# nz0001na/MorphGANformer

Hardware: AMD Instinct MI355X
Metric: latent-projection iters/sec @1024^2, k=17 latents (higher is better)
Workload: dtype f32; 1 GPU; configs[1]: single 1024x1024 face per GPU, Wing+LPIPS(squeeze)+MSE literal-mode projection step, noise_mode=random, seeded synthetic weights/targets/landmarks; k=17, z_dim=32, targets_per_gpu=1, parallelism=pair-sharded x1, graph_replay=True, loss_generator_overlap=True, steps_per_forward=32

## Files before the change

### include/mgf.h

```cpp
#ifndef MGF_H_
#define MGF_H_

#include <stdint.h>

#ifdef __cplusplus
extern "C" {
#endif

typedef void* mgf_stream_t;

enum { MGF_OK = 0, MGF_EINVAL = -1, MGF_EUNSUPPORTED = -2, MGF_ELAUNCH = -3, MGF_ETOOBIG = -4 };
enum { MGF_F32 = 0, MGF_F64 = 1, MGF_F16 = 2 };
enum { MGF_FILTER_SEPARABLE = 2 };
enum { MGF_FILTER_LARGE = 4 };
enum { MGF_ACT_LINEAR = 1, MGF_ACT_RELU = 2, MGF_ACT_LRELU = 3, MGF_ACT_TANH = 4, MGF_ACT_SIGMOID = 5,
       MGF_ACT_ELU = 6, MGF_ACT_SELU = 7, MGF_ACT_SOFTPLUS = 8, MGF_ACT_SWISH = 9,
       MGF_ACT_RELU_POST = 10 };

const char* mgf_last_error(void);
int mgf_version(void);
int mgf_device_ok(void);

int mgf_bias_act(void* y, const void* x, const void* b, const void* xref, const void* yref, const void* dy,
                 int dtype, int64_t numel, int64_t step_b, int64_t size_b,
// ... 121 lines not shown
} mgf_style_job;
int mgf_demod_f32(float* d, const float* s, const float* wsq, int32_t n, int32_t cin, int32_t cout, mgf_stream_t stream);
int mgf_demod_bwd_f32(float* ds, const float* dd, const float* d, const float* s, const float* wsq, int32_t n, int32_t cin, int32_t cout,
                      mgf_stream_t stream);
int mgf_style_demod(const mgf_style_job* job, const float* ws, int64_t ws_stride_n, int32_t n, int32_t wdim, mgf_stream_t stream);
int mgf_style_demod_multi(const mgf_style_job* jobs_dev, int32_t njobs, const float* ws, int64_t ws_stride_n,
                          int32_t n, int32_t wdim, int32_t max_cin, mgf_stream_t stream);

int mgf_duplex_attention(float* y, const float* x, const float* wqc, const float* spos, const float* vwb,
                         int32_t n, int32_t c, int32_t f, int32_t t,
                         const mgf_epilogue* ep, int32_t ep_w, float* probs, int32_t* argmax, mgf_stream_t stream);

int mgf_att_map_upsample_f32(float* out, const float* probs, int32_t n, int32_t side, int32_t t, int32_t out_res, int32_t layer,
                             int32_t n_layers, mgf_stream_t stream);

typedef struct mgf_attn_job {
    const float* wmv;
    const float* bmv;
    float* vwb;
    int32_t c;
    int32_t w_offset;
} mgf_attn_job;
int mgf_attn_values(const mgf_attn_job* job, const float* ws, int64_t ws_stride_n, int64_t ws_stride_t, int32_t n, int32_t t,
                    int32_t wdim, mgf_stream_t stream);
int mgf_attn_values_multi(const mgf_attn_job* jobs_dev, int32_t njobs, const float* ws, int64_t ws_stride_n, int64_t ws_stride_t,
                          int32_t n, int32_t t, int32_t wdim, mgf_stream_t stream);

int mgf_randn_f32(float* out, int64_t n, uint64_t seed, void* state, mgf_stream_t stream);
int mgf_rgb_weights_f32(float* out, const float* w, const float* s, int32_t n, int32_t c, int32_t cout, mgf_stream_t stream);
int mgf_torgb_compose_weights_f32(float* w_eff, const float* w_last, const float* s_last, const float* d_last, const float* w_rgb,
                                  const float* s_rgb, int32_t n, int32_t cin, int32_t cout, int32_t rgb_channels, mgf_stream_t stream);
int mgf_conv3x3_few_outputs_f32(float* y, const float* x, const float* w, const float* bias, int32_t n, int32_t cin, int32_t h, int32_t wd,
                                int32_t cout, mgf_stream_t stream);

int64_t mgf_mapping_param_floats(int32_t k, int32_t dim, int32_t n_res_layers);
int mgf_mapping_forward(float* w, const float* z, const float* params, int32_t n, int32_t k, int32_t dim,
                        int32_t n_res_layers, int32_t normalize_global, mgf_stream_t stream);

int64_t mgf_reduce_scratch_floats(void);
int mgf_mse_f32(float* out, const float* a, const float* b, int32_t n, int64_t numel, int64_t b_batch_stride, float scale,
                int32_t accumulate, float* scratch, mgf_stream_t stream);
int64_t mgf_dssim_scratch_bytes(int32_t n, int32_t c, int32_t h, int32_t w);
int mgf_dssim_u8_f32(float* out, const float* img, const float* target, int32_t n, int32_t c, int32_t h, int32_t w, int64_t t_batch_stride,
                     float data_range, float scale, int32_t accumulate, void* scratch, mgf_stream_t stream);
int mgf_dssim_f32(float* out, const float* img, const float* target, int32_t n, int32_t c, int32_t h, int32_t w, int64_t t_batch_stride,
                  float data_range, float scale, int32_t accumulate, void* scratch, mgf_stream_t stream);
int mgf_dssim_grad_f32(float* dimg, float* out, const float* img, const float* target, int32_t n, int32_t c, int32_t h, int32_t w,
                       int64_t t_batch_stride, float data_range, float scale, int32_t accumulate_dimg, int32_t accumulate_out, void* scratch,
                       mgf_stream_t stream);
int64_t mgf_msssim_scratch_bytes(int32_t n, int32_t c, int32_t h, int32_t w, int32_t levels);
int mgf_msssim_f32(float* out, const float* img, const float* target, int32_t n, int32_t c, int32_t h, int32_t w, int64_t t_batch_stride,
                   const double* weights, int32_t levels, float data_range, float scale, int32_t accumulate, void* scratch, mgf_stream_t stream);
int mgf_msssim_grad_f32(float* dimg, float* out, const float* img, const float* target, int32_t n, int32_t c, int32_t h, int32_t w,
                        int64_t t_batch_stride, const double* weights, int32_t levels, float data_range, float scale, int32_t accumulate_dimg,
                        int32_t accumulate_out, void* scratch, mgf_stream_t stream);
int64_t mgf_lbp_scratch_bytes(int32_t n);
int mgf_lbp_gray224_u8(uint8_t* gray, const float* img, const int32_t* tables, int32_t n, int32_t h, int32_t w, int32_t true_rgb_order,
                       mgf_stream_t stream);
int mgf_lbp_codes_u8(uint8_t* codes, const uint8_t* gray, const double* offsets, int32_t n, mgf_stream_t stream);
int mgf_lbp_distance_f64(double* out, const uint8_t* gray, const uint8_t* target_codes, const double* offsets, int32_t n, void* scratch,
                         mgf_stream_t stream);
int mgf_wing_loss_f64(double* out, const double* pred, const double* target, int32_t n, int64_t numel, double omega, double epsilon,
                      const int32_t* pred_step, int32_t max_row, mgf_stream_t stream);
int mgf_adaptive_wing_loss_f64(double* out, const double* pred, const double* target, int32_t n, int64_t numel, double omega, double theta,
                               double epsilon, double alpha, const int32_t* pred_step, int32_t max_row, mgf_stream_t stream);
int mgf_embed_pair_loss_f32(float* loss, float* demb, double* trace, const float* emb, const float* ta, const float* tb, const float* alpha,
// ... 199 lines not shown
```

### morphganformer_amd/_lib.py

```python
from __future__ import annotations

import ctypes as C
import os

import torch

HERE = os.path.dirname(os.path.abspath(__file__))
LIB_PATH = os.environ.get("MGF_LIB_PATH") or os.path.join(HERE, "libmgf_hip.so")

MGF_F32, MGF_F64, MGF_F16 = 0, 1, 2
ACT_IDS = {"linear": 1, "relu": 2, "lrelu": 3, "tanh": 4, "sigmoid": 5, "elu": 6, "selu": 7, "softplus": 8, "swish": 9,
           "relu_post": 10}
MAX_TAPS = 9

i32, i64, f32, f64, vp = C.c_int32, C.c_int64, C.c_float, C.c_double, C.c_void_p


class Epilogue(C.Structure):
    _fields_ = [("bias", vp), ("noise", vp), ("noise_strength", vp), ("noise_n", i32), ("act", i32), ("alpha", f32),
                ("gain", f32), ("residual", vp)]


class ConvDesc(C.Structure):
    _fields_ = [("n", i32), ("cin", i32), ("in_h", i32), ("in_w", i32), ("cout", i32), ("cout_pad", i32),
# ... 44 lines not shown
    "mgf_tconv3x3s2_blur_f32": (C.c_int, [vp, vp, vp, vp, vp, vp, C.c_float, i32, i32, i32, i32, i32, i32, i64, i64, i64, i64, C.POINTER(Epilogue), vp]),
    "mgf_tconv3x3s2_winograd_f32": (C.c_int, [vp, vp, vp, vp, vp, i32, i32, i32, i32, i32, i32, i64, i64, i64, vp]),
    "mgf_tconv_winograd_weights_f32": (C.c_int, [vp, vp, i32, i32, C.c_double, vp]),
    "mgf_winograd_weights_f32": (C.c_int, [vp, vp, i32, i32, f32, vp]),
    "mgf_conv3x3_winograd_f32": (C.c_int, [vp, vp, vp, vp, vp, i32, i32, i32, i32, i32, i32, C.POINTER(Epilogue), vp]),
    "mgf_winograd2_weights_f32": (C.c_int, [vp, vp, i32, i32, f32, vp]),
    "mgf_conv3x3_winograd2_f32": (C.c_int, [vp, vp, vp, vp, vp, i32, i32, i32, i32, i32, i32, C.POINTER(Epilogue), vp]),
    "mgf_conv3x3_winograd2_rgb_f32": (C.c_int, [vp, vp, vp, vp, vp, vp, vp, i32, i32, i32, i32, i32, i32, i32, vp]),
    "mgf_conv3x3_winograd3_f32": (C.c_int, [vp, vp, vp, vp, vp, i32, i32, i32, i32, i32, i32, C.POINTER(Epilogue), vp]),
    "mgf_conv1x1_f32": (C.c_int, [vp, vp, vp, vp, i32, i32, i32, i32, i32, i64, i32, C.POINTER(Epilogue), vp]),
    "mgf_conv3x3s2_few_inputs_f32": (C.c_int, [vp, vp, vp, vp, i32, i32, i32, i32, i32, i32, vp]),
    "mgf_tconv3x3s2_few_outputs_f32": (C.c_int, [vp, vp, vp, i32, i32, i32, i32, i32, i32, i32, i64, i64, vp]),
    "mgf_conv1x1_force_shape": (C.c_int, [i32]),
    "mgf_conv3x3_winograd3_slice_f32": (C.c_int, [vp, vp, vp, vp, vp, i32, i32, i32, i32, i32, i32, i64, i32, C.POINTER(Epilogue), vp]),
    "mgf_conv3x3_winograd3_up2res_f32": (C.c_int, [vp, vp, vp, vp, vp, vp, i32, i32, i32, i32, i32, i32, C.POINTER(Epilogue), vp]),
    "mgf_winograd3_force_shape": (C.c_int, [i32]),
    "mgf_conv3x3_winograd3_rgb_f32": (C.c_int, [vp, vp, vp, vp, vp, vp, vp, i32, i32, i32, i32, i32, i32, i32, vp]),
    "mgf_conv3x3_winograd2_slice_f32": (C.c_int, [vp, vp, vp, vp, vp, i32, i32, i32, i32, i32, i32, i64, i32, C.POINTER(Epilogue), vp]),
    "mgf_pack_conv_weights": (C.c_int, [vp, vp, vp, i32, i32, i32, i32, i32, f32, i32, vp]),
    "mgf_conv_profile_begin": (C.c_int, []),
    "mgf_conv_profile_end": (C.c_int, [C.POINTER(ConvProfRec), i32]),
    "mgf_demod_f32": (C.c_int, [vp, vp, vp, i32, i32, i32, vp]),
    "mgf_demod_bwd_f32": (C.c_int, [vp, vp, vp, vp, vp, i32, i32, i32, vp]),
    "mgf_style_demod": (C.c_int, [C.POINTER(StyleJob), vp, i64, i32, i32, vp]),
    "mgf_style_demod_multi": (C.c_int, [vp, i32, vp, i64, i32, i32, i32, vp]),
    "mgf_duplex_attention": (C.c_int, [vp, vp, vp, vp, vp, i32, i32, i32, i32, C.POINTER(Epilogue), i32, vp, vp, vp]),
    "mgf_att_map_upsample_f32": (C.c_int, [vp, vp, i32, i32, i32, i32, i32, i32, vp]),
    "mgf_attn_values": (C.c_int, [C.POINTER(AttnJob), vp, i64, i64, i32, i32, i32, vp]),
    "mgf_attn_values_multi": (C.c_int, [vp, i32, vp, i64, i64, i32, i32, i32, vp]),
    "mgf_randn_f32": (C.c_int, [vp, i64, C.c_uint64, vp, vp]),
    "mgf_rgb_weights_f32": (C.c_int, [vp, vp, vp, i32, i32, i32, vp]),
    "mgf_torgb_compose_weights_f32": (C.c_int, [vp, vp, vp, vp, vp, vp, i32, i32, i32, i32, vp]),
    "mgf_conv3x3_few_outputs_f32": (C.c_int, [vp, vp, vp, vp, i32, i32, i32, i32, i32, vp]),
    "mgf_mapping_param_floats": (i64, [i32, i32, i32]),
    "mgf_mapping_forward": (C.c_int, [vp, vp, vp, i32, i32, i32, i32, i32, vp]),
    "mgf_reduce_scratch_floats": (i64, []),
    "mgf_mse_f32": (C.c_int, [vp, vp, vp, i32, i64, i64, f32, i32, vp, vp]),
    "mgf_dssim_scratch_bytes": (i64, [i32, i32, i32, i32]),
    "mgf_dssim_u8_f32": (C.c_int, [vp, vp, vp, i32, i32, i32, i32, i64, f32, f32, i32, vp, vp]),
    "mgf_dssim_f32": (C.c_int, [vp, vp, vp, i32, i32, i32, i32, i64, f32, f32, i32, vp, vp]),
    "mgf_dssim_grad_f32": (C.c_int, [vp, vp, vp, vp, i32, i32, i32, i32, i64, f32, f32, i32, i32, vp, vp]),
    "mgf_msssim_scratch_bytes": (i64, [i32, i32, i32, i32, i32]),
    "mgf_msssim_f32": (C.c_int, [vp, vp, vp, i32, i32, i32, i32, i64, vp, i32, f32, f32, i32, vp, vp]),
    "mgf_msssim_grad_f32": (C.c_int, [vp, vp, vp, vp, i32, i32, i32, i32, i64, vp, i32, f32, f32, i32, i32, vp, vp]),
    "mgf_lbp_scratch_bytes": (i64, [i32]),
    "mgf_lbp_gray224_u8": (C.c_int, [vp, vp, vp, i32, i32, i32, i32, vp]),
    "mgf_lbp_codes_u8": (C.c_int, [vp, vp, vp, i32, vp]),
    "mgf_lbp_distance_f64": (C.c_int, [vp, vp, vp, vp, i32, vp, vp]),
    "mgf_wing_loss_f64": (C.c_int, [vp, vp, vp, i32, i64, f64, f64, vp, i32, vp]),
    "mgf_adaptive_wing_loss_f64": (C.c_int, [vp, vp, vp, i32, i64, f64, f64, f64, f64, vp, i32, vp]),
    "mgf_embed_pair_loss_f32": (C.c_int, [vp, vp, vp, vp, vp, vp, vp, i32, i32, i64, f32, f32, i32, i32, vp, i32, vp]),
    "mgf_lpips_unit_f32": (C.c_int, [vp, vp, i32, i32, i64, vp]),
    "mgf_lpips_layer_f32": (C.c_int, [vp, vp, vp, vp, i32, i32, i64, i64, i32, vp, vp]),
    "mgf_lpips_stem_f32": (C.c_int, [vp, vp, vp, vp, vp, vp, vp, vp, i32, i32, i32, i32, vp, vp]),
    "mgf_lpips_layer_map_f32": (C.c_int, [vp, vp, vp, vp, i32, i32, i64, i64, vp]),
    "mgf_lpips_upsample_sum_f32": (C.c_int, [vp, C.POINTER(vp), C.POINTER(i32), i32, i32, i32, i32, vp]),
    "mgf_channel_affine_prelu_f32":(C.c_int, [vp, vp, vp, vp, vp, i32, i32, i64, vp]),
    "mgf_linear_f32": (C.c_int, [vp, vp, vp, vp, i32, i32, i32, vp]),
    "mgf_resize_bilinear_f32": (C.c_int, [vp, vp, i32, i32, i32, i32, i32, vp]),
    "mgf_spatial_mean_f32": (C.c_int, [vp, vp, i32, i64, vp]),
    "mgf_l2_normalize_f32": (C.c_int, [vp, vp, i32, i32, f32, vp]),
    "mgf_l2_normalize_bwd_f32": (C.c_int, [vp, vp, vp, i32, i32, f32, vp]),
    "mgf_spatial_mean_bwd_f32": (C.c_int, [vp, vp, i32, i64, vp]),
    "mgf_relu_bwd_slice_f32": (C.c_int, [vp, vp, i32, i32, vp, i32, i32, i32, i32, i64, vp]),
    "mgf_maxpool_s2_floor_f32": (C.c_int, [vp, vp, i32, i32, i32, i32, vp]),
    "mgf_maxpool3x3s2_ceil_f32": (C.c_int, [vp, vp, i32, i32, i32, i32, i32, vp]),
# ... 129 lines not shown
```

### morphganformer_amd/build.py

```python
from __future__ import annotations

import glob
import hashlib
import os
import subprocess
import sys

HERE = os.path.dirname(os.path.abspath(__file__))
ROOT = os.path.dirname(HERE)
CSRC = os.path.join(HERE, "csrc")
OBJ = os.path.join(CSRC, "_obj")
LIB = os.path.join(HERE, "libmgf_hip.so")
SOURCES = ["capi.cpp", "bias_act.hip", "upfirdn2d.hip", "conv_taps.hip", "latent_prep.hip", "attention.hip", "losses.hip", "lpips_stem.hip",
           "embed.hip", "backward.hip", "wino.hip", "wino3.hip", "pointwise.hip", "narrow_conv.hip", "warp.hip", "lbp.hip", "mdf.hip",
           "wino_tconv.hip", "depthwise.hip", "noise_opt.hip", "morph_pair.hip", "tconv_blur.hip", "msssim.hip"]
HEADERS = [os.path.join(CSRC, "mgf_common.h"), os.path.join(ROOT, "include", "mgf.h")]
HIPCC = os.environ.get("HIPCC", "/opt/rocm/bin/hipcc")
FLAGS = ["--offload-arch=gfx950", "-O3", "-fPIC", "-std=c++17", "-ffp-contract=on", "-Wno-unused-result", "-x", "hip"]
LINK_FLAGS = ["--offload-arch=gfx950", "-shared", "-fPIC"]

_compiler_id = None


def compiler_id() -> str:
    global _compiler_id
    if _compiler_id is None:
        _compiler_id = subprocess.run([HIPCC, "--version"], stdout=subprocess.PIPE, stderr=subprocess.STDOUT, check=True).stdout.decode()
    return _compiler_id


def object_key(src_path: str, flags) -> str:
    h = hashlib.sha256()
    h.update(compiler_id().encode())
    h.update("\0".join(flags).encode())
    for p in [src_path] + HEADERS:
        with open(p, "rb") as f:
            h.update(b"\0" + os.path.basename(p).encode() + b"\0" + f.read())
    return h.hexdigest()[:16]


def _compile_all(obj_dir, flags_for, verbose, force, prune=True):
    os.makedirs(obj_dir, exist_ok=True)
    objs, todo = [], []
    for src in SOURCES:
        sp = os.path.join(CSRC, src)
        flags = flags_for(src)
        op = os.path.join(obj_dir, f"{src}.{object_key(sp, flags)}.o")
        objs.append(op)
# ... 95 lines not shown
```

### morphganformer_amd/conv.py

```python
from __future__ import annotations

import ctypes as C
import os
from dataclasses import dataclass

import torch

from . import _lib


def round_up(v: int, m: int) -> int:
    return (v + m - 1) // m * m


def profile_begin():
    _lib.check(_lib.lib().mgf_conv_profile_begin(), "conv_profile_begin")


def profile_end(max_recs=4096):
    recs = (_lib.ConvProfRec * max_recs)()
    n = _lib.lib().mgf_conv_profile_end(recs, max_recs)
    if n < 0:
        _lib.check(n, "conv_profile_end")
    return [(recs[i].kernel.decode(), recs[i].flops, recs[i].seconds, recs[i].ksplit, recs[i].bytes) for i in range(min(n, max_recs))]


@dataclass
class PackedConv:
    wp: torch.Tensor
    wsq: torch.Tensor | None
    cout: int
    cin: int
    kh: int
    kw: int
    cout_pad: int
# ... 328 lines not shown

def tconv_pitch(w: int, align: int = 4) -> int:
    return round_up(2 * w + 1, align)


def conv3x3s2_few_inputs(x, w, bias=None, relu=False, out=None):
    _lib.require_gpu(x, w, bias, out)
    cout, cin = w.shape[:2]
    assert tuple(w.shape[2:]) == (3, 3) and cin <= 4 and w.is_contiguous() and w.dtype == torch.float32
    assert x.dtype == torch.float32 and x.is_contiguous() and x.shape[1] == cin
    n, _, h, wd = x.shape
    oh, ow = (h - 3) // 2 + 1, (wd - 3) // 2 + 1
    if out is None:
        out = torch.empty([n, cout, oh, ow], dtype=torch.float32, device=x.device)
    assert out.is_contiguous() and tuple(out.shape) == (n, cout, oh, ow)
    rc = _lib.lib().mgf_conv3x3s2_few_inputs_f32(out.data_ptr(), x.data_ptr(), w.data_ptr(), _lib.ptr(bias), n, cin, h, wd, cout, int(relu),
                                                 _lib.stream_ptr())
    _lib.check(rc, "conv3x3s2_few_inputs")
    return out


def conv3x3_few_outputs(x, w, bias=None, out=None):
    _lib.require_gpu(x, w, bias, out)
    n, cin, h, wd = x.shape
    cout = w.shape[1]
    assert x.dtype == torch.float32 and x.is_contiguous() and w.dtype == torch.float32 and w.is_contiguous()
    assert tuple(w.shape) == (n, cout, cin, 3, 3) and cout <= 4
    if out is None:
        out = torch.empty([n, cout, h, wd], dtype=torch.float32, device=x.device)
    assert out.is_contiguous() and tuple(out.shape) == (n, cout, h, wd)
    _lib.check(_lib.lib().mgf_conv3x3_few_outputs_f32(out.data_ptr(), x.data_ptr(), w.data_ptr(), _lib.ptr(bias), n, cin, h, wd, cout,
                                                      _lib.stream_ptr()), "conv3x3_few_outputs")
    return out


TCONV_WINO = os.environ.get("MGF_TCONV_WINO", "1") != "0"
TCONV_WINO_MIN_WGS = 4096


def tconv_winograd_weights(w: torch.Tensor, gain: float = 1.0) -> torch.Tensor:
    _lib.require_gpu(w)
    w = w.contiguous().float()
    cout, cin, kh, kw = w.shape
    assert (kh, kw) == (3, 3) and cin % 4 == 0
    u = torch.empty([25, cin // 4, cout, 4], dtype=torch.float32, device=w.device)
    _lib.check(_lib.lib().mgf_tconv_winograd_weights_f32(u.data_ptr(), w.data_ptr(), cout, cin, float(gain), _lib.stream_ptr()),
               "tconv_winograd_weights")
    return u


def tconv_winograd_ok(n, cin, h, w, cout, out, bf=None) -> bool:
    return bool(TCONV_WINO and SPLIT_TCONV_BORDER and bf is None and h % 2 == 0 and w % 2 == 0 and min(h, w) >= TCONV_SPLIT_MIN and cin % 4 == 0 and cout % 32 == 0
                and out.shape[3] % 4 == 0 and out.data_ptr() % 16 == 0
                and n * -(-h // 4) * -(-w // 32) * (cout // 32) >= TCONV_WINO_MIN_WGS)


def tconv3x3s2_forward(x, pc: PackedConv, in_scale=None, out_scale=None, out=None, bf=None, wt=None):
    _lib.require_gpu(x, pc.wp, in_scale, out_scale, out, wt)
    assert pc.kh == 3 and pc.kw == 3 and x.dtype == torch.float32 and x.is_contiguous()
    n, cin, h, w = x.shape
    oh, ow = 2 * h + 1, 2 * w + 1
    if out is None:
        out = torch.empty([n, pc.cout, oh, tconv_pitch(w)], dtype=torch.float32, device=x.device)
    pitch = out.shape[3]
    assert out.is_contiguous() and tuple(out.shape) == (n, pc.cout, oh, pitch) and pitch >= ow and pitch % 4 == 0
    if NARROW_CONV and pc.cout <= 4 and in_scale is None and out_scale is None:
# ... 106 lines not shown
```

### morphganformer_amd/engine.py

```python
from __future__ import annotations

import ctypes as C
import math
import os
from dataclasses import dataclass, field

import numpy as np
import torch

from . import _lib
from . import conv as cv
from .synth_weights import GeneratorConfig

SQRT2 = math.sqrt(2.0)
SQRT_HALF = math.sqrt(0.5)
USE_WINOGRAD = os.environ.get("MGF_WINOGRAD", "1") != "0"
WINOGRAD_MAX_RES = int(os.environ.get("MGF_WINOGRAD_MAX_RES", "1024"))
TCONV_WINO_MAX_RES = int(os.environ.get("MGF_TCONV_WINO_MAX_RES", "256"))
BF_DIRECT_MAX_RES = int(os.environ.get("MGF_BF_DIRECT_MAX_RES", "128"))


def pack_mapping_params(sd, cfg: GeneratorConfig) -> np.ndarray:
    D, T = cfg.w_dim, cfg.k - 1
    lr = cfg.mapping_lrmul
# ... 102 lines not shown
                lp.demod = False
            else:
                wg = 1.0 / math.sqrt(cin * 9)
                lp.pc = cv.pack_weights(t32(w), gain=wg, flip=False, want_wsq=True)
                if kind == "conv3" and USE_WINOGRAD and cv.winograd_ok(cin, cout, res, res) and res <= WINOGRAD_MAX_RES:
                    lp.wino_u = cv.winograd_pack(t32(w), wg, res)
                if (kind == "tconv" and arith != "bf16x3" and cv.TCONV_WINO and res <= TCONV_WINO_MAX_RES and cin % 4 == 0
                        and cout % 32 == 0):
                    lp.wino_t = cv.tconv_winograd_weights(t32(w), wg)
                if arith == "bf16x3" and cin % 16 == 0 and res // up >= 32:
                    lp.pcb = cv.pack_weights_bf16x3(lp.pc)
            lp.aff_w = t32(f64(p + ".affine.weight"))
            lp.aff_b = t32(f64(p + ".affine.bias"))
            if (p + ".biasAct.bias") in sd:
                lp.bias = t32(f64(p + ".biasAct.bias"))
            if (p + ".noise_strength") in sd:
                lp.noise_strength = t32(f64(p + ".noise_strength").reshape(1))
                lp.noise_const = t32(f64(p + ".noise_const"))
            lp.act_gain = SQRT2 * (SQRT_HALF if (name == "conv1" and res > 4) else 1.0)
            if att and (p + ".transformer.to_queries.weight") in sd:
                lp.attn = self._fold_attention(sd, p, cout, res, T, D, t32, f64)
                lp.attn.v_off = v_off
                v_off += cout * T
            if name == "conv_last" and lp.bias is None and lp.noise_strength is None and lp.attn is None and cfg.img_channels <= 4:
                lp.w_gained = t32(w / math.sqrt(cin * 9))
            lp.s_off, lp.d_off = s_off, d_off
            s_off += cin
            d_off += cout
            self.layers.append(lp)
        self.s_total, self.d_total, self.v_total = s_off, d_off, v_off
        for res in cfg.block_resolutions[1:]:
            w = f64(f"synthesis.b{res}.skip.weight")
            self.skips[res] = cv.pack_weights(t32(w), gain=SQRT_HALF / math.sqrt(w.shape[1]), flip=False)
        torch.cuda.synchronize(dev)

    @staticmethod
    def _fold_attention(sd, p, C_, res, T, D, t32, f64):
        tp = p + ".transformer"
        Fn = res * res
        wq = f64(tp + ".to_queries.weight") / math.sqrt(C_)
        bq = f64(tp + ".to_queries.bias")
        wfp = f64(tp + ".from_pos_map.weight") / math.sqrt(D)
        bfp = f64(tp + ".from_pos_map.bias")
        wv = f64(tp + ".to_values.weight") / math.sqrt(D)
        bv = f64(tp + ".to_values.bias")
        wm = f64(tp + ".modulation.weight") / math.sqrt(C_)
        bm = f64(tp + ".modulation.bias")
        aw = f64(tp + ".att_weight").reshape(2 * C_)
        cent = f64(tp + ".centroids").reshape(T, 2 * C_)
        a1 = cent[:, :C_] * aw[None, :C_]
        a2 = cent[:, C_:] * aw[None, C_:]
        inv = 1.0 / math.sqrt(C_)
        wqc = (wq.T @ a1.T) * inv
        pos_term = f64(p + ".grid_pos").reshape(Fn, D) @ wfp.T + bfp[None]
        spos = (pos_term @ a2.T + (bq @ a1.T)[None]) * inv
        wmv = wm @ wv
        bmv = wm @ bv + bm + 1.0
        return AttnPlan(c=C_, f=Fn, wqc=t32(wqc), spos=t32(spos), wmv=t32(wmv), bmv=t32(bmv))


class Generator:

    def __init__(self, sd, cfg: GeneratorConfig, device="cuda", max_batch: int = 1, arith: str = "f32"):
        if arith not in ("f32", "bf16x3"):
            raise ValueError(f"arith must be 'f32' or 'bf16x3' (got {arith!r})")
        self.cfg = cfg
        self.arith = arith
        self.tpitch_align = 32 if arith == "bf16x3" else 4
        self.plan = SynthesisPlan(sd, cfg, device, arith=arith)
        self.device = self.plan.device
        self.input_shape = [None, cfg.k, cfg.z_dim]
        self.cond_shape = [None, 0]
        self.z_dim, self.w_dim, self.k, self.c_dim = cfg.z_dim, cfg.w_dim, cfg.k, 0
        self.img_resolution, self.img_channels = cfg.img_resolution, cfg.img_channels
        self.num_ws = cfg.num_ws
        self.w_avg = torch.as_tensor(np.asarray(sd["mapping.w_avg"], dtype=np.float32), device=self.device)
        self._ws_cache = {}
        self.taps = None
        self.fuse_torgb = True
        self.skip_fused = {}
        self.fuse_skip_up = os.environ.get("MGF_FUSE_SKIP_UP", "1") != "0"
        self.last_noise = ("none", None)
        self.side = torch.cuda.Stream(device=self.device)
        self.overlap_skip = os.environ.get("MGF_OVERLAP_SKIP", "0") != "0"
        self.torgb_compose = os.environ.get("MGF_TORGB_COMPOSE", "1") != "0"
        self._workspaces, self._pins = {}, {}
        self.noise_seed, self._noise_epoch = int(torch.initial_seed()) & 0xFFFFFFFFFFFFFFFF, None
        self.noise_state = torch.zeros(2, dtype=torch.int64, device=self.device)
        self._alloc(max_batch)

    _WS_FIELDS = ("n", "lean", "w_buf", "styles", "demods", "vtabs", "noise_rand", "bufs", "img", "const_in", "rgbw", "w_eff", "style_jobs", "n_style_jobs",
                  "max_style_cin", "attn_jobs", "n_attn_jobs", "style_jobs_pl", "attn_jobs_pl", "ws_bytes", "ws_gen")

    def _alloc(self, n, lean=None):
        cur = (getattr(self, "n", None), getattr(self, "lean", False))
        lean = cur[1] if lean is None else bool(lean)
        if cur[0] is not None and cur in self._workspaces:
            self._workspaces[cur]["noise_rand"] = self.noise_rand
        key = (n, lean)
        ws = self._workspaces.pop(key, None)
        if ws is None:
            self._evict_for(n, lean)
            self._create(n, lean)
            ws = {k: getattr(self, k) for k in self._WS_FIELDS}
        self._workspaces[key] = ws
        for k, v in ws.items():
            setattr(self, k, v)

    def pin(self, key=None):
        key = (self.n, self.lean) if key is None else key
        self._pins[key] = self._pins.get(key, 0) + 1
        return key

    def unpin(self, key):
        if self._pins.get(key, 0) > 0:
            self._pins[key] -= 1

    def _evict_for(self, n, lean):
        budget = float(os.environ.get("MGF_WORKSPACE_GB", "160")) * 2 ** 30
        need = self._workspace_bytes(n, lean)
        total = sum(w["ws_bytes"] for w in self._workspaces.values())
        cur = (getattr(self, "n", None), getattr(self, "lean", False))
        for m in list(self._workspaces):
            if total + need <= budget:
                break
            if self._pins.get(m, 0) == 0 and m != cur:
                total -= self._workspaces.pop(m)["ws_bytes"]

    def _fuses_skip_up(self, l1, n):
        res = l1.res
        if l1.pcb is not None and res <= BF_DIRECT_MAX_RES:
            return False
        return bool(self.fuse_skip_up and self.plan.fir_is_1331 and cv.WINOGRAD_FORM == 3 and l1.attn is None and l1.wino_u is not None
                    and l1.wino_u.ndim == 4 and res % 2 == 0 and cv.winograd_fills_chip(n, l1.cout, res, res))

    def _lean_arenas(self, n):
        cfg = self.cfg
        conv1 = {lp.res: lp for lp in self.plan.layers if lp.name.endswith(".conv1")}
        a = dict(T=0, U=0, V=0, W0=0, W1=0, S=0, SL=0)
        for i, res in enumerate(cfg.block_resolutions):
            c, px = cfg.channels(res), res * res
            a["U"] = max(a["U"], c * px)
            a["W%d" % (i & 1)] = max(a["W%d" % (i & 1)], c * px)
            if res > 4:
                a["T"] = max(a["T"], c * (res + 1) * cv.tconv_pitch(res // 2, self.tpitch_align))
                a["SL"] = max(a["SL"], c * px // 4)
                if not self._fuses_skip_up(conv1[res], n):
                    a["S"] = max(a["S"], c * px)
                if cfg.has_attention(res):
                    a["V"] = max(a["V"], c * px)
            if res == cfg.img_resolution:
                a["T"] = max(a["T"], c * px)
        return a

    def _workspace_bytes(self, n, lean=False):
        cfg = self.cfg
        if lean:
            return 4 * n * (sum(self._lean_arenas(n).values()) + cfg.img_channels * cfg.img_resolution ** 2)
        per = 0
        for res in cfg.block_resolutions:
            c = cfg.channels(res)
            planes = 1 + (4 if res > 4 else 0) + (1 if res > 4 and cfg.has_attention(res) else 0) + (1 if cfg.has_attention(res) else 0) \
                + (1 if res == cfg.img_resolution else 0)
            per += planes * c * res * res
        return 4 * n * (per + cfg.img_channels * cfg.img_resolution ** 2)

    def _create(self, n, lean=False):
        cfg, dev, P = self.cfg, self.device, self.plan
        e = lambda *s: torch.empty(s, dtype=torch.float32, device=dev)
        self.n, self.lean = n, bool(lean)
        self._gen_counter = getattr(self, "_gen_counter", 0) + 1
        self.ws_gen = self._gen_counter
        self.w_buf = e(n, cfg.k, cfg.w_dim)
        self.styles = e(n, P.s_total)
        self.demods = e(n, P.d_total)
        self.vtabs = e(n, max(P.v_total, 1))
        self.noise_rand = None
        self.bufs = {}
        if lean:
            arena = {k: e(n * v) for k, v in self._lean_arenas(n).items() if v}
            conv1 = {lp.res: lp for lp in P.layers if lp.name.endswith(".conv1")}
            view = lambda k, *shape: arena[k][:int(np.prod(shape))].view(*shape)
            for i, res in enumerate(cfg.block_resolutions):
                c, att, W = cfg.channels(res), cfg.has_attention(res), "W%d" % (i & 1)
                b = {"conv1": view("U" if att else W, n, c, res, res)}
                if att:
                    b["conv1a"] = view(W, n, c, res, res)
                if res > 4:
                    b["skip_low"] = view("SL", n, c, res // 2, res // 2)
                    b["t"] = view("T", n, c, res + 1, cv.tconv_pitch(res // 2, self.tpitch_align))
                    b["conv0"] = view("U", n, c, res, res)
                    if att:
                        b["conv0a"] = view("V", n, c, res, res)
                    if not self._fuses_skip_up(conv1[res], n):
                        b["skip"] = view("S", n, c, res, res)
                if res == cfg.img_resolution:
                    b["last"] = view("T", n, c, res, res)
                self.bufs[res] = b
        for res in ([] if lean else cfg.block_resolutions):
            c = cfg.channels(res)
            b = {"conv1": e(n, c, res, res)}
            if res > 4:
                b["skip_low"] = e(n, c, res // 2, res // 2)
                b["skip"] = e(n, c, res, res)
                b["t"] = e(n, c, res + 1, cv.tconv_pitch(res // 2, self.tpitch_align))
                b["conv0"] = e(n, c, res, res)
                if cfg.has_attention(res):
                    b["conv0a"] = e(n, c, res, res)
            if cfg.has_attention(res):
                b["conv1a"] = e(n, c, res, res)
            if res == cfg.img_resolution:
                b["last"] = e(n, c, res, res)
            self.bufs[res] = b
        self.img = e(n, cfg.img_channels, cfg.img_resolution, cfg.img_resolution)
        self.const_in = P.const.unsqueeze(0).repeat(n, 1, 1, 1).contiguous()
        self.rgbw = e(n, cfg.img_channels, cfg.channels(cfg.img_resolution))
        self.w_eff = e(n, cfg.img_channels, cfg.channels(cfg.img_resolution), 3, 3)
        self.ws_bytes = self._workspace_bytes(n, lean)
        self._build_jobs(n)

    def _build_jobs(self, n):
        cfg, P = self.cfg, self.plan
        D, NW = cfg.w_dim, cfg.num_ws

        def tables(per_layer):
            sj = (_lib.StyleJob * len(P.layers))()
            aj = []
            for i, lp in enumerate(P.layers):
                g_off = ((cfg.k - 1) * NW + lp.slot) * D if per_layer else (cfg.k - 1) * D
                sj[i] = _lib.StyleJob(lp.aff_w.data_ptr(), lp.aff_b.data_ptr(), _lib.ptr(lp.pc.wsq) if lp.demod else 0,
                                      self.styles.data_ptr() + 4 * lp.s_off * n,
                                      (self.demods.data_ptr() + 4 * lp.d_off * n) if lp.demod else 0,
                                      lp.cin, lp.cout, g_off, 1.0 / math.sqrt(D), lp.style_gain)
                if lp.attn is not None:
                    aj.append(_lib.AttnJob(lp.attn.wmv.data_ptr(), lp.attn.bmv.data_ptr(),
                                           self.vtabs.data_ptr() + 4 * lp.attn.v_off * n, lp.attn.c, lp.slot * D if per_layer else 0))
            sjt = torch.frombuffer(bytearray(bytes(sj)), dtype=torch.uint8).to(self.device)
            ajt = None
            if aj:
                arr = (_lib.AttnJob * len(aj))(*aj)
                ajt = torch.frombuffer(bytearray(bytes(arr)), dtype=torch.uint8).to(self.device)
            return sjt, ajt, len(aj)

        self.style_jobs, self.attn_jobs, self.n_attn_jobs = tables(False)
        self.style_jobs_pl, self.attn_jobs_pl, _ = tables(True)
        self.n_style_jobs = len(P.layers)
        self.max_style_cin = max(lp.cin for lp in P.layers)

    def _s(self, lp):
        return self.styles.view(-1)[lp.s_off * self.n:(lp.s_off + lp.cin) * self.n].view(self.n, lp.cin)
# ... 77 lines not shown
        if n != self.n:
            raise _lib.MgfError("synthesis: batch size changed; call through __call__ / mapping first")
        if self.lean and (self.taps is not None or return_att):
            self._alloc(n, False)
        st = _lib.stream_ptr()
        D, T = cfg.w_dim, cfg.k - 1
        _lib.require_gpu(w)
        per_layer = w.ndim == 4
        if per_layer:
            if tuple(w.shape) != (n, cfg.k, cfg.num_ws, D):
                raise _lib.MgfError(f"synthesis: ws must be [n, {cfg.k}, {cfg.num_ws}, {D}] (got {tuple(w.shape)})")
            w = w.contiguous().float()
            stride_n, stride_t = cfg.k * cfg.num_ws * D, cfg.num_ws * D
            sjobs, ajobs = self.style_jobs_pl, self.attn_jobs_pl
        else:
            assert w.is_contiguous() and tuple(w.shape) == (n, cfg.k, D)
            stride_n, stride_t = cfg.k * D, D
            sjobs, ajobs = self.style_jobs, self.attn_jobs
        self.last_w = w
        _lib.check(L.mgf_style_demod_multi(sjobs.data_ptr(), self.n_style_jobs, w.data_ptr(), stride_n, n, D, self.max_style_cin, st),
                   "style_demod_multi")
        if self.n_attn_jobs:
            _lib.check(L.mgf_attn_values_multi(ajobs.data_ptr(), self.n_attn_jobs, w.data_ptr(), stride_n, stride_t, n, T, D, st),
                       "attn_values_multi")
        if noise_mode == "random":
            noises = self._draw_noise(n)
        self.last_noise = (noise_mode, noises)
        layers = {lp.name: lp for lp in P.layers}
        self.att_maps = {} if return_att else None
        x = None
        for res in cfg.block_resolutions:
            b = f"synthesis.b{res}"
            B = self.bufs[res]
            if res == 4:
                x_in = self.const_in
                x = self._layer(layers[b + ".conv1"], x_in, B, "conv1", noise_mode, noises, residual=None)
            else:
                l1 = layers[b + ".conv1"]
                fuse_up = self._fuses_skip_up(l1, n)
                if not fuse_up and "skip" not in B:
                    raise _lib.MgfError(f"synthesis: the lean workspace has no full-resolution skip tensor for the {res}x{res} block "
                                        "(fuse_skip_up changed after the workspace was created): use the full workspace")
                self.skip_fused[res] = bool(fuse_up)
                main = torch.cuda.current_stream(self.device)
                if self.overlap_skip:
                    self.side.wait_stream(main)
                    with torch.cuda.stream(self.side):
                        cv.conv_forward(x, P.skips[res], out=B["skip_low"])
                        if not fuse_up:
                            cv.upfirdn_into(B["skip"], B["skip_low"], P.fir, up=2, pad=(2, 1, 2, 1), gain=4.0, separable=True)
                else:
                    cv.conv_forward(x, P.skips[res], out=B["skip_low"])
                    if not fuse_up:
                        cv.upfirdn_into(B["skip"], B["skip_low"], P.fir, up=2, pad=(2, 1, 2, 1), gain=4.0, separable=True)
                x0 = self._layer(layers[b + ".conv0"], x, B, "conv0", noise_mode, noises, residual=None)
                if self.overlap_skip:
                    main.wait_stream(self.side)
                if fuse_up:
                    x = self._layer(l1, x0, B, "conv1", noise_mode, noises, residual=None, residual_low=B["skip_low"])
                else:
                    x = self._layer(l1, x0, B, "conv1", noise_mode, noises, residual=B["skip"])
            if self.taps is not None:
                self.taps[b] = x
            if res == cfg.img_resolution:
                lp = layers[b + ".conv_last"]
                lt = layers[b + ".torgb"]
                if self.taps is None and self.fuse_torgb and self.torgb_compose and lp.w_gained is not None:
                    _lib.check(L.mgf_torgb_compose_weights_f32(self.w_eff.data_ptr(), lp.w_gained.data_ptr(), self._s(lp).data_ptr(),
                                                               self._d(lp).data_ptr(), lt.w_raw.data_ptr(), self._s(lt).data_ptr(), n, lp.cin,
                                                               lp.cout, lt.w_raw.shape[0], st), "torgb_compose_weights")
                    cv.conv3x3_few_outputs(x, self.w_eff, lt.bias, out=self.img)
                elif self.taps is None and self.fuse_torgb and lp.cout <= 32:
                    _lib.check(L.mgf_rgb_weights_f32(self.rgbw.data_ptr(), lt.w_raw.data_ptr(), self._s(lt).data_ptr(), n, lt.w_raw.shape[0],
                                                     lt.w_raw.shape[1], st), "rgb_weights")
                    if lp.wino_u is not None and lp.wino_u.ndim == 4 and lp.cout == 32 and cv.winograd_fills_chip(n, lp.cout, res, res):
                        cv.winograd2_rgb_forward(x, lp.wino_u, self.rgbw, lt.bias, self.img, in_scale=self._s(lp), out_scale=self._d(lp))
                    else:
                        cv.conv_forward(x, lp.pc, pad=(1, 1), in_scale=self._s(lp), out_scale=self._d(lp),
                                        rgb=(self.rgbw, lt.bias, self.img))
                else:
                    if lp.wino_u is not None and cv.winograd_fills_chip(n, lp.cout, res, res):
                        x = cv.winograd_forward(x, lp.wino_u, in_scale=self._s(lp), out_scale=self._d(lp), out=B["last"])
                    else:
                        x = cv.conv_forward(x, lp.pc, pad=(1, 1), in_scale=self._s(lp), out_scale=self._d(lp), out=B["last"])
                    if self.taps is not None:
                        self.taps[b] = x
                    ep = _lib.make_epilogue(bias=lt.bias)
                    cv.conv_forward(x, lt.pc, in_scale=self._s(lt), epilogue=ep, out=self.img)
        return self.img

    def list2tensor(self, att_maps=None):
        att_maps = self.att_maps if att_maps is None else att_maps
        if not att_maps:
            return torch.zeros([1], device=self.device)
        T, R = self.cfg.k - 1, self.cfg.img_resolution
        names = [lp.name for lp in self.plan.layers if lp.name in att_maps]
        n = att_maps[names[0]][0].shape[0]
        out = torch.empty([n, T, len(names), 1, R, R], dtype=torch.float32, device=self.device)
        for i, name in enumerate(names):
            probs = att_maps[name][0]
            side = math.isqrt(probs.shape[1])
            _lib.check(_lib.lib().mgf_att_map_upsample_f32(out.data_ptr(), probs.data_ptr(), n, side, T, R, i, len(names),
                                                           _lib.stream_ptr()), "att_map_upsample")
        return out
# ... 123 lines not shown
```

Baseline: 800.1 iters/s.

## Fold final-block skip path through composed toRGB into a direct image add

```diff
diff --git a/include/mgf.h b/include/mgf.h
--- a/include/mgf.h
+++ b/include/mgf.h
@@ -177,6 +177,10 @@
                                   const float* s_rgb, int32_t n, int32_t cin, int32_t cout, int32_t rgb_channels, mgf_stream_t stream);
 int mgf_conv3x3_few_outputs_f32(float* y, const float* x, const float* w, const float* bias, int32_t n, int32_t cin, int32_t h, int32_t wd,
                                 int32_t cout, mgf_stream_t stream);
+int mgf_skip_rgb_compose_weights_f32(float* m, const float* w_eff, const float* p, int32_t n, int32_t rgb_channels, int32_t cmid,
+                                     int32_t cin, mgf_stream_t stream);
+int mgf_skip_rgb_add_f32(float* img, const float* x, const float* m, int32_t n, int32_t cin, int32_t h, int32_t w, int32_t channels,
+                         float e0, float e1, float o0, float o1, mgf_stream_t stream);
 
 int64_t mgf_mapping_param_floats(int32_t k, int32_t dim, int32_t n_res_layers);
 int mgf_mapping_forward(float* w, const float* z, const float* params, int32_t n, int32_t k, int32_t dim,
diff --git a/morphganformer_amd/_lib.py b/morphganformer_amd/_lib.py
--- a/morphganformer_amd/_lib.py
+++ b/morphganformer_amd/_lib.py
@@ -100,6 +100,8 @@
     "mgf_rgb_weights_f32": (C.c_int, [vp, vp, vp, i32, i32, i32, vp]),
     "mgf_torgb_compose_weights_f32": (C.c_int, [vp, vp, vp, vp, vp, vp, i32, i32, i32, i32, vp]),
     "mgf_conv3x3_few_outputs_f32": (C.c_int, [vp, vp, vp, vp, i32, i32, i32, i32, i32, vp]),
+    "mgf_skip_rgb_compose_weights_f32": (C.c_int, [vp, vp, vp, i32, i32, i32, i32, vp]),
+    "mgf_skip_rgb_add_f32": (C.c_int, [vp, vp, vp, i32, i32, i32, i32, i32, f32, f32, f32, f32, vp]),
     "mgf_mapping_param_floats": (i64, [i32, i32, i32]),
     "mgf_mapping_forward": (C.c_int, [vp, vp, vp, i32, i32, i32, i32, i32, vp]),
     "mgf_reduce_scratch_floats": (i64, []),
diff --git a/morphganformer_amd/build.py b/morphganformer_amd/build.py
--- a/morphganformer_amd/build.py
+++ b/morphganformer_amd/build.py
@@ -13,7 +13,7 @@
 LIB = os.path.join(HERE, "libmgf_hip.so")
 SOURCES = ["capi.cpp", "bias_act.hip", "upfirdn2d.hip", "conv_taps.hip", "latent_prep.hip", "attention.hip", "losses.hip", "lpips_stem.hip",
            "embed.hip", "backward.hip", "wino.hip", "wino3.hip", "pointwise.hip", "narrow_conv.hip", "warp.hip", "lbp.hip", "mdf.hip",
-           "wino_tconv.hip", "depthwise.hip", "noise_opt.hip", "morph_pair.hip", "tconv_blur.hip", "msssim.hip"]
+           "wino_tconv.hip", "depthwise.hip", "noise_opt.hip", "morph_pair.hip", "tconv_blur.hip", "msssim.hip", "skip_rgb.hip"]
 HEADERS = [os.path.join(CSRC, "mgf_common.h"), os.path.join(ROOT, "include", "mgf.h")]
 HIPCC = os.environ.get("HIPCC", "/opt/rocm/bin/hipcc")
 FLAGS = ["--offload-arch=gfx950", "-O3", "-fPIC", "-std=c++17", "-ffp-contract=on", "-Wno-unused-result", "-x", "hip"]
diff --git a/morphganformer_amd/conv.py b/morphganformer_amd/conv.py
--- a/morphganformer_amd/conv.py
+++ b/morphganformer_amd/conv.py
@@ -1,6 +1,7 @@
 from __future__ import annotations
 
 import ctypes as C
+import math
 import os
 from dataclasses import dataclass
 
@@ -395,6 +396,38 @@
     _lib.check(_lib.lib().mgf_conv3x3_few_outputs_f32(out.data_ptr(), x.data_ptr(), w.data_ptr(), _lib.ptr(bias), n, cin, h, wd, cout,
                                                       _lib.stream_ptr()), "conv3x3_few_outputs")
     return out
+
+
+def skip_rgb_weights(w_eff, p, out=None):
+    _lib.require_gpu(w_eff, p, out)
+    n, rc, cmid = w_eff.shape[:3]
+    cin = p.shape[1]
+    assert w_eff.dtype == torch.float32 and w_eff.is_contiguous() and tuple(w_eff.shape[3:]) == (3, 3)
+    assert p.dtype == torch.float32 and p.is_contiguous() and tuple(p.shape) == (cmid, cin)
+    if out is None:
+        out = torch.empty([n, cin, 9, rc], dtype=torch.float32, device=w_eff.device)
+    assert out.is_contiguous() and tuple(out.shape) == (n, cin, 9, rc)
+    _lib.check(_lib.lib().mgf_skip_rgb_compose_weights_f32(out.data_ptr(), w_eff.data_ptr(), p.data_ptr(), n, rc, cmid, cin, _lib.stream_ptr()),
+               "skip_rgb_compose_weights")
+    return out
+
+
+def skip_rgb_taps(f1d, gain=4.0):
+    g = [float(v) * math.sqrt(gain) for v in f1d.detach().double().cpu()]
+    assert len(g) == 4
+    return g[3], g[1], g[2], g[0]
+
+
+def skip_rgb_add(img, x, m, taps):
+    _lib.require_gpu(img, x, m)
+    n, cin, h, w = x.shape
+    rc = img.shape[1]
+    assert x.dtype == torch.float32 and x.is_contiguous() and m.dtype == torch.float32 and m.is_contiguous()
+    assert img.dtype == torch.float32 and img.is_contiguous() and tuple(img.shape) == (n, rc, 2 * h, 2 * w) and rc <= 4
+    assert tuple(m.shape) == (n, cin, 9, rc) and cin % 8 == 0
+    _lib.check(_lib.lib().mgf_skip_rgb_add_f32(img.data_ptr(), x.data_ptr(), m.data_ptr(), n, cin, h, w, rc, *[float(t) for t in taps],
+                                               _lib.stream_ptr()), "skip_rgb_add")
+    return img
 
 
 TCONV_WINO = os.environ.get("MGF_TCONV_WINO", "1") != "0"
diff --git a/morphganformer_amd/csrc/skip_rgb.hip b/morphganformer_amd/csrc/skip_rgb.hip
--- /dev/null
+++ b/morphganformer_amd/csrc/skip_rgb.hip
@@ -0,0 +1,228 @@
+#include <algorithm>
+
+#include "mgf_common.h"
+
+namespace {
+
+typedef const float __attribute__((address_space(4)))* sr_cfp;
+typedef float sr_f2 __attribute__((ext_vector_type(2)));
+
+constexpr int SR_MAX_CO = 4;
+constexpr int SR_OWN_LANES = MGF_WAVE - 2;
+constexpr int SR_CH = 4;
+
+struct sr_taps { float e0, e1, o0, o1; };
+
+template <bool VEC>
+__device__ __forceinline__ sr_f2 sr_load(const float* row, int qa, int qb, bool oka, bool okb) {
+    sr_f2 v;
+    if (VEC) {
+        v = *reinterpret_cast<const sr_f2*>(row + qa);
+    } else {
+        v.x = row[qa];
+        v.y = row[qb];
+    }
+    v.x = oka ? v.x : 0.f;
+    v.y = okb ? v.y : 0.f;
+    return v;
+}
+
+__device__ __forceinline__ void sr_fold(float& even, float& odd, float m_l, float z_l, float m, float z, float p, float z_r, float p_r,
+                                        const sr_taps t, float cl, float cr) {
+    float e = t.o0 * m_l;
+    e = fmaf(cl, m, e);
+    e = fmaf(t.e0, z_l, e);
+    e = fmaf(t.e1, z, e);
+    e = fmaf(t.o0, p, e);
+    even = fmaf(t.o1, p_r, e);
+    float o = t.e0 * m_l;
+    o = fmaf(t.e1, m, o);
+    o = fmaf(t.o0, z, o);
+    o = fmaf(t.o1, z_r, o);
+    o = fmaf(cr, p, o);
+    odd = fmaf(t.e1, p_r, o);
+}
+
+template <int NT>
+__device__ __forceinline__ void sr_mac(sr_f2 (&v)[NT], const sr_f2 (&xs)[SR_CH], float (&mw)[NT], sr_cfp mn, int c0, int cin) {
+#pragma unroll
+    for (int k = 0; k < SR_CH; ++k) {
+        if (NT <= 27) {
+            const int cn = c0 + k + 1 == cin ? 0 : c0 + k + 1;
+            const sr_cfp mc = mn + cn * NT;
+            float nx[NT];
+#pragma unroll
+            for (int i = 0; i < NT; ++i) nx[i] = mc[i];
+#pragma unroll
+            for (int i = 0; i < NT; ++i) v[i] = __builtin_elementwise_fma(sr_f2{mw[i], mw[i]}, xs[k], v[i]);
+#pragma unroll
+            for (int i = 0; i < NT; ++i) mw[i] = nx[i];
+        } else {
+            const sr_cfp mc = mn + (c0 + k) * NT;
+#pragma unroll
+            for (int i = 0; i < NT; ++i) {
+                const float mv = mc[i];
+                v[i] = __builtin_elementwise_fma(sr_f2{mv, mv}, xs[k], v[i]);
+            }
+        }
+    }
+}
+
+template <int CO, bool VEC>
+__global__ __launch_bounds__(MGF_WAVE) void skip_rgb_kernel(float* __restrict__ img, const float* __restrict__ x, const float* m, int cin,
+                                                            int h, int w, int rows, sr_taps t) {
+    constexpr int NT = 9 * CO;
+    const int lane = threadIdx.x;
+    const int n = blockIdx.z, r0 = blockIdx.y * rows, r1 = min(r0 + rows, h);
+    const int q0 = (int)blockIdx.x * (2 * SR_OWN_LANES) - 2 + 2 * lane;
+    const bool own = lane >= 1 && lane <= SR_OWN_LANES && q0 < w;
+    const int64_t plane = (int64_t)h * w;
+    const float* xn = x + (int64_t)n * cin * plane;
+    const sr_cfp mn = (sr_cfp)m + (int64_t)n * cin * NT;
+    const int w2 = 2 * w;
+    float* yb = img + (int64_t)n * CO * 4 * plane;
+    float* yn = yb + 2 * q0;
+    const float clA = q0 > 0 ? t.o1 : 0.f, crA = q0 < w - 1 ? t.e0 : 0.f;
+    const float clB = q0 + 1 > 0 ? t.o1 : 0.f, crB = q0 + 1 < w - 1 ? t.e0 : 0.f;
+
+    float accE[CO][4], accO[CO][4], preE[CO][4], preO[CO][4];
+#pragma unroll
+    for (int c = 0; c < CO; ++c)
+#pragma unroll
+        for (int k = 0; k < 4; ++k) accE[c][k] = accO[c][k] = preE[c][k] = preO[c][k] = 0.f;
+
+    float mw[NT];
+#pragma unroll
+    for (int i = 0; i < NT; ++i) mw[i] = mn[i];
+    const bool inA = q0 >= 0 && q0 < w, inB = q0 + 1 >= 0 && q0 + 1 < w;
+    const int qa = VEC ? min(max(q0, 0), w - 2) : min(max(q0, 0), w - 1), qb = min(max(q0 + 1, 0), w - 1);
+    sr_f2 xa[SR_CH], xb[SR_CH];
+    {
+        const int r = r0 - 1;
+        const bool ok = r >= 0;
+        const float* xr = xn + (int64_t)max(r, 0) * w;
+#pragma unroll
+        for (int k = 0; k < SR_CH; ++k) xa[k] = sr_load<VEC>(xr + k * plane, qa, qb, ok && inA, ok && inB);
+    }
+    for (int r = r0 - 1; r <= r1; ++r) {
+        const bool row_ok = r >= 0 && r < h, next_ok = r + 1 < h;
+        const float* xr = xn + (int64_t)min(max(r, 0), h - 1) * w;
+        const float* xnext = xn + (int64_t)min(r + 1, h - 1) * w;
+        sr_f2 v[NT];
+#pragma unroll
+        for (int i = 0; i < NT; ++i) v[i] = sr_f2{0.f, 0.f};
+        for (int c0 = 0; c0 < cin; c0 += 2 * SR_CH) {
+#pragma unroll
+            for (int k = 0; k < SR_CH; ++k) xb[k] = sr_load<VEC>(xr + (c0 + SR_CH + k) * plane, qa, qb, row_ok && inA, row_ok && inB);
+            sr_mac<NT>(v, xa, mw, mn, c0, cin);
+            const bool last = c0 + 2 * SR_CH >= cin;
+            const float* xf = last ? xnext : xr + (c0 + 2 * SR_CH) * plane;
+            const bool ok = last ? next_ok : row_ok;
+#pragma unroll
+            for (int k = 0; k < SR_CH; ++k) xa[k] = sr_load<VEC>(xf + k * plane, qa, qb, ok && inA, ok && inB);
+            sr_mac<NT>(v, xb, mw, mn, c0 + SR_CH, cin);
+        }
+        const float cu = r > 0 ? t.o1 : 0.f, cd = r < h - 1 ? t.e0 : 0.f;
+        const bool store = own && r - 1 >= r0;
+        float4 ie[CO], io[CO];
+        if (VEC) {
+            const float* yl = yb + (int64_t)(2 * max(r - 1, 0)) * w2 + min(max(2 * q0, 0), w2 - 4);
+#pragma unroll
+            for (int c = 0; c < CO; ++c) {
+                ie[c] = *reinterpret_cast<const float4*>(yl + (int64_t)c * 2 * h * w2);
+                io[c] = *reinterpret_cast<const float4*>(yl + (int64_t)c * 2 * h * w2 + w2);
+            }
+        }
+#pragma unroll
+        for (int c = 0; c < CO; ++c) {
+            float hz[3][4];
+#pragma unroll
+            for (int kh = 0; kh < 3; ++kh) {
+                const sr_f2 vm = v[(kh * 3 + 0) * CO + c], vz = v[(kh * 3 + 1) * CO + c], vp = v[(kh * 3 + 2) * CO + c];
+                const float lm = __shfl_up(vm.y, 1, MGF_WAVE), lz = __shfl_up(vz.y, 1, MGF_WAVE);
+                const float rz = __shfl_down(vz.x, 1, MGF_WAVE), rp = __shfl_down(vp.x, 1, MGF_WAVE);
+                sr_fold(hz[kh][0], hz[kh][1], lm, lz, vm.x, vz.x, vp.x, vz.y, vp.y, t, clA, crA);
+                sr_fold(hz[kh][2], hz[kh][3], vm.x, vz.x, vm.y, vz.y, vp.y, rz, rp, t, clB, crB);
+            }
+            float oe[4], oo[4];
+#pragma unroll
+            for (int k = 0; k < 4; ++k) {
+                const float hm = hz[0][k], hc = hz[1][k], hp = hz[2][k];
+                oe[k] = fmaf(t.o1, hp, accE[c][k]);
+                oo[k] = fmaf(t.e1, hp, fmaf(t.o1, hc, accO[c][k]));
+                accE[c][k] = fmaf(t.o0, hp, fmaf(t.e1, hc, fmaf(cu, hm, preE[c][k])));
+                accO[c][k] = fmaf(cd, hp, fmaf(t.o0, hc, fmaf(t.e1, hm, preO[c][k])));
+                preE[c][k] = fmaf(t.e0, hc, t.o0 * hm);
+                preO[c][k] = t.e0 * hm;
+            }
+            if (store) {
+                float* ye = yn + ((int64_t)c * 2 * h + 2 * (r - 1)) * w2;
+                float* yo = ye + w2;
+                if (VEC) {
+                    float4 a = ie[c], b = io[c];
+                    a.x += oe[0]; a.y += oe[1]; a.z += oe[2]; a.w += oe[3];
+                    b.x += oo[0]; b.y += oo[1]; b.z += oo[2]; b.w += oo[3];
+                    *reinterpret_cast<float4*>(ye) = a;
+                    *reinterpret_cast<float4*>(yo) = b;
+                } else {
+#pragma unroll
+                    for (int k = 0; k < 4; ++k)
+                        if (2 * q0 + k < w2) {
+                            ye[k] += oe[k];
+                            yo[k] += oo[k];
+                        }
+                }
+            }
+        }
+    }
+}
+
+__global__ __launch_bounds__(256) void skip_rgb_compose_kernel(float* out, const float* w_eff, const float* p, int rc, int cmid, int cin, int total) {
+    const int i = blockIdx.x * 256 + threadIdx.x;
+    if (i >= total) return;
+    const int c = i % rc, d = (i / rc) % 9, ci = (i / (9 * rc)) % cin, n = i / (9 * rc * cin);
+    double acc = 0.0;
+    for (int s = 0; s < cmid; ++s) acc += (double)w_eff[(((int64_t)n * rc + c) * cmid + s) * 9 + d] * (double)p[(int64_t)s * cin + ci];
+    out[i] = (float)acc;
+}
+
+}
+
+extern "C" int mgf_skip_rgb_compose_weights_f32(float* m, const float* w_eff, const float* p, int32_t n, int32_t rgb_channels, int32_t cmid,
+                                                int32_t cin, mgf_stream_t stream) {
+    MGF_REQUIRE(m && w_eff && p && n >= 1 && rgb_channels >= 1 && cmid >= 1 && cin >= 1, MGF_EINVAL, "skip_rgb_compose_weights: bad arguments");
+    MGF_REQUIRE((int64_t)n * rgb_channels * cin * 9 <= INT32_MAX && (int64_t)n * rgb_channels * cmid * 9 <= INT32_MAX && (int64_t)cmid * cin <= INT32_MAX,
+                MGF_ETOOBIG, "skip_rgb_compose_weights: too many weights");
+    const int total = n * rgb_channels * cin * 9;
+    hipLaunchKernelGGL(skip_rgb_compose_kernel, dim3((unsigned)mgf_cdiv(total, 256)), dim3(256), 0, (hipStream_t)stream, m, w_eff, p,
+                       rgb_channels, cmid, cin, total);
+    MGF_CHECK_LAUNCH("skip_rgb_compose_weights");
+    return MGF_OK;
+}
+
+extern "C" int mgf_skip_rgb_add_f32(float* img, const float* x, const float* m, int32_t n, int32_t cin, int32_t h, int32_t w,
+                                    int32_t channels, float e0, float e1, float o0, float o1, mgf_stream_t stream) {
+    MGF_REQUIRE(img && x && m && n >= 1 && cin >= 1 && h >= 1 && w >= 1, MGF_EINVAL, "skip_rgb_add: bad arguments");
+    MGF_REQUIRE(channels >= 1 && channels <= SR_MAX_CO, MGF_EUNSUPPORTED, "skip_rgb_add: 1..%d image channels (got %d)", SR_MAX_CO, channels);
+    MGF_REQUIRE(cin % (2 * SR_CH) == 0, MGF_EUNSUPPORTED, "skip_rgb_add: the input channel count must be a multiple of %d (got %d)", 2 * SR_CH, cin);
+    MGF_REQUIRE(n <= 65535 && w <= (INT32_MAX - 8) / 2 && (int64_t)cin * 9 * channels <= INT32_MAX, MGF_ETOOBIG, "skip_rgb_add: tensor too large");
+    const int gx = (int)mgf_cdiv(w, 2 * SR_OWN_LANES);
+    const int64_t strips = std::max<int64_t>(1, (int64_t)8 * MGF_NUM_CU / ((int64_t)n * gx));
+    int rows = (int)std::max<int64_t>(4, mgf_cdiv(h, strips));
+    static const char* rows_env = mgf_knob("MGF_SKIP_RGB_ROWS");
+    if (rows_env) rows = std::max(1, atoi(rows_env));
+    MGF_REQUIRE(mgf_cdiv(h, rows) <= 65535, MGF_ETOOBIG, "skip_rgb_add: map too tall");
+    const bool vec = w % 2 == 0 && ((uintptr_t)x % 8) == 0 && ((uintptr_t)img % 16) == 0;
+    const dim3 grid((unsigned)gx, (unsigned)mgf_cdiv(h, rows), (unsigned)n);
+    const sr_taps t{e0, e1, o0, o1};
+    hipStream_t st = (hipStream_t)stream;
+#define MGF_SR_LAUNCH(CO)                                                                                                          \
+    do {                                                                                                                           \
+        if (vec) hipLaunchKernelGGL((skip_rgb_kernel<CO, true>), grid, dim3(MGF_WAVE), 0, st, img, x, m, cin, h, w, rows, t);      \
+        else hipLaunchKernelGGL((skip_rgb_kernel<CO, false>), grid, dim3(MGF_WAVE), 0, st, img, x, m, cin, h, w, rows, t);         \
+    } while (0)
+    if (channels == 1) MGF_SR_LAUNCH(1); else if (channels == 2) MGF_SR_LAUNCH(2); else if (channels == 3) MGF_SR_LAUNCH(3); else MGF_SR_LAUNCH(4);
+#undef MGF_SR_LAUNCH
+    MGF_CHECK_LAUNCH("skip_rgb_add");
+    return MGF_OK;
+}
diff --git a/morphganformer_amd/engine.py b/morphganformer_amd/engine.py
--- a/morphganformer_amd/engine.py
+++ b/morphganformer_amd/engine.py
@@ -158,6 +158,11 @@
         for res in cfg.block_resolutions[1:]:
             w = f64(f"synthesis.b{res}.skip.weight")
             self.skips[res] = cv.pack_weights(t32(w), gain=SQRT_HALF / math.sqrt(w.shape[1]), flip=False)
+        self.skip_rgb_w = self.skip_rgb_taps = None
+        if len(cfg.block_resolutions) > 1 and self.fir1 is not None:
+            w = f64(f"synthesis.b{cfg.img_resolution}.skip.weight")
+            self.skip_rgb_w = t32(w.reshape(w.shape[0], w.shape[1]) * (SQRT_HALF / math.sqrt(w.shape[1])))
+            self.skip_rgb_taps = cv.skip_rgb_taps(self.fir1, 4.0)
         torch.cuda.synchronize(dev)
 
     @staticmethod
@@ -210,12 +215,13 @@
         self.side = torch.cuda.Stream(device=self.device)
         self.overlap_skip = os.environ.get("MGF_OVERLAP_SKIP", "0") != "0"
         self.torgb_compose = os.environ.get("MGF_TORGB_COMPOSE", "1") != "0"
+        self.skip_rgb = os.environ.get("MGF_SKIP_RGB", "1") != "0"
         self._workspaces, self._pins = {}, {}
         self.noise_seed, self._noise_epoch = int(torch.initial_seed()) & 0xFFFFFFFFFFFFFFFF, None
         self.noise_state = torch.zeros(2, dtype=torch.int64, device=self.device)
         self._alloc(max_batch)
 
-    _WS_FIELDS = ("n", "lean", "w_buf", "styles", "demods", "vtabs", "noise_rand", "bufs", "img", "const_in", "rgbw", "w_eff", "style_jobs", "n_style_jobs",
+    _WS_FIELDS = ("n", "lean", "w_buf", "styles", "demods", "vtabs", "noise_rand", "bufs", "img", "const_in", "rgbw", "w_eff", "skip_m", "style_jobs", "n_style_jobs",
                   "max_style_cin", "attn_jobs", "n_attn_jobs", "style_jobs_pl", "attn_jobs_pl", "ws_bytes", "ws_gen")
 
     def _alloc(self, n, lean=None):
@@ -260,6 +266,16 @@
         return bool(self.fuse_skip_up and self.plan.fir_is_1331 and cv.WINOGRAD_FORM == 3 and l1.attn is None and l1.wino_u is not None
                     and l1.wino_u.ndim == 4 and res % 2 == 0 and cv.winograd_fills_chip(n, l1.cout, res, res))
 
+    def _skip_to_image(self):
+        cfg, P = self.cfg, self.plan
+        res = cfg.img_resolution
+        if not self.skip_rgb or P.skip_rgb_w is None or not P.fir_is_1331 or self.taps is not None:
+            return False
+        lp = next(l for l in P.layers if l.name == f"synthesis.b{res}.conv_last")
+        l1 = next(l for l in P.layers if l.name == f"synthesis.b{res}.conv1")
+        return bool(self.fuse_torgb and self.torgb_compose and lp.w_gained is not None and l1.attn is None
+                    and P.skip_rgb_w.shape[1] % 8 == 0 and cfg.img_channels <= 4)
+
     def _lean_arenas(self, n):
         cfg = self.cfg
         conv1 = {lp.res: lp for lp in self.plan.layers if lp.name.endswith(".conv1")}
@@ -270,9 +286,10 @@
             a["W%d" % (i & 1)] = max(a["W%d" % (i & 1)], c * px)
             if res > 4:
                 a["T"] = max(a["T"], c * (res + 1) * cv.tconv_pitch(res // 2, self.tpitch_align))
-                a["SL"] = max(a["SL"], c * px // 4)
-                if not self._fuses_skip_up(conv1[res], n):
-                    a["S"] = max(a["S"], c * px)
+                if not (res == cfg.img_resolution and self._skip_to_image()):
+                    a["SL"] = max(a["SL"], c * px // 4)
+                    if not self._fuses_skip_up(conv1[res], n):
+                        a["S"] = max(a["S"], c * px)
                 if cfg.has_attention(res):
                     a["V"] = max(a["V"], c * px)
             if res == cfg.img_resolution:
@@ -313,13 +330,14 @@
                 if att:
                     b["conv1a"] = view(W, n, c, res, res)
                 if res > 4:
-                    b["skip_low"] = view("SL", n, c, res // 2, res // 2)
                     b["t"] = view("T", n, c, res + 1, cv.tconv_pitch(res // 2, self.tpitch_align))
                     b["conv0"] = view("U", n, c, res, res)
                     if att:
                         b["conv0a"] = view("V", n, c, res, res)
-                    if not self._fuses_skip_up(conv1[res], n):
-                        b["skip"] = view("S", n, c, res, res)
+                    if not (res == cfg.img_resolution and self._skip_to_image()):
+                        b["skip_low"] = view("SL", n, c, res // 2, res // 2)
+                        if not self._fuses_skip_up(conv1[res], n):
+                            b["skip"] = view("S", n, c, res, res)
                 if res == cfg.img_resolution:
                     b["last"] = view("T", n, c, res, res)
                 self.bufs[res] = b
@@ -342,6 +360,7 @@
         self.const_in = P.const.unsqueeze(0).repeat(n, 1, 1, 1).contiguous()
         self.rgbw = e(n, cfg.img_channels, cfg.channels(cfg.img_resolution))
         self.w_eff = e(n, cfg.img_channels, cfg.channels(cfg.img_resolution), 3, 3)
+        self.skip_m = e(n, P.skip_rgb_w.shape[1], 9, cfg.img_channels) if P.skip_rgb_w is not None else None
         self.ws_bytes = self._workspace_bytes(n, lean)
         self._build_jobs(n)
 
@@ -485,12 +504,20 @@
         for res in cfg.block_resolutions:
             b = f"synthesis.b{res}"
             B = self.bufs[res]
+            rgb_skip = res == cfg.img_resolution and res > 4 and self._skip_to_image()
             if res == 4:
                 x_in = self.const_in
                 x = self._layer(layers[b + ".conv1"], x_in, B, "conv1", noise_mode, noises, residual=None)
+            elif rgb_skip:
+                x_low = x
+                x0 = self._layer(layers[b + ".conv0"], x, B, "conv0", noise_mode, noises, residual=None)
+                x = self._layer(layers[b + ".conv1"], x0, B, "conv1", noise_mode, noises, residual=None)
             else:
                 l1 = layers[b + ".conv1"]
                 fuse_up = self._fuses_skip_up(l1, n)
+                if "skip_low" not in B:
+                    raise _lib.MgfError(f"synthesis: the lean workspace has no skip tensor for the {res}x{res} block (skip_rgb / torgb_compose "
+                                        "changed after the workspace was created): use the full workspace")
                 if not fuse_up and "skip" not in B:
                     raise _lib.MgfError(f"synthesis: the lean workspace has no full-resolution skip tensor for the {res}x{res} block "
                                         "(fuse_skip_up changed after the workspace was created): use the full workspace")
@@ -523,6 +550,9 @@
                                                                self._d(lp).data_ptr(), lt.w_raw.data_ptr(), self._s(lt).data_ptr(), n, lp.cin,
                                                                lp.cout, lt.w_raw.shape[0], st), "torgb_compose_weights")
                     cv.conv3x3_few_outputs(x, self.w_eff, lt.bias, out=self.img)
+                    if rgb_skip:
+                        cv.skip_rgb_weights(self.w_eff, P.skip_rgb_w, out=self.skip_m)
+                        cv.skip_rgb_add(self.img, x_low, self.skip_m, P.skip_rgb_taps)
                 elif self.taps is None and self.fuse_torgb and lp.cout <= 32:
                     _lib.check(L.mgf_rgb_weights_f32(self.rgbw.data_ptr(), lt.w_raw.data_ptr(), self._s(lt).data_ptr(), n, lt.w_raw.shape[0],
                                                      lt.w_raw.shape[1], st), "rgb_weights")
```

Result: no change. 799.7 iters/s (median of 2 runs) (-0.0%).
